# Gericom/MobiclipDecoder

Measured on AMD Instinct MI355X. Metric: decoded Mpixels/s @ 640x480 P-frames, higher is better.
Workload: dtype u8

## Files before the change

### mobiclipdecoder_amd/csrc/mobi_kernels.hip

```cpp
#include <hip/hip_runtime.h>
#include <stdint.h>
#include <stdlib.h>

#include <type_traits>

#include "mobi_cmd.h"
#include "mobi_kernels.h"
#include "mobi_recon_math.h"
#include "mobi_tile.h"

namespace {

enum { TP = 32 };

__device__ __forceinline__ void wave_sync() { __builtin_amdgcn_fence(__ATOMIC_ACQ_REL, "wavefront"); }

struct Geo {
  int width, height, stride, mbw, lg;
  __device__ __forceinline__ int owner_luma(int a) const {
    if (a < 0) return -1;
    const int row = a >> lg, col = a & (stride - 1);
    if (col >= width || row >= height) return -1;
    return (row >> 4) * mbw + (col >> 4);
  }
// ... 235 lines not shown
  const uint32_t pA[2] = {*(const uint32_t *)waA, *(const uint32_t *)wbA}, pB[2] = {*(const uint32_t *)waB, *(const uint32_t *)wbB};
  uint32_t resA[2], resB[2];
#pragma unroll
  for (int h = 0; h < 2; h++) {
    uint32_t sat[4];
#pragma unroll
    for (int k = 0; k < 4; k++) {
      const s16x2 pp = __builtin_bit_cast(s16x2, __builtin_amdgcn_perm(pB[h], pA[h], 0x0c040c00u + (uint32_t)k * 0x00010001u));
      const s16x2 sum = __builtin_elementwise_add_sat(pp, out[4 * h + k] >> (short)6);
      lo = __builtin_elementwise_min(lo, sum);
      hi = __builtin_elementwise_max(hi, sum);
      sat[k] = sat_pk_u8(sum);
    }
    const uint32_t m01 = __builtin_amdgcn_perm(sat[1], sat[0], 0x05010400u), m23 = __builtin_amdgcn_perm(sat[3], sat[2], 0x05010400u);
    resA[h] = __builtin_amdgcn_perm(m23, m01, 0x05040100u);
    resB[h] = __builtin_amdgcn_perm(m23, m01, 0x07060302u);
  }
  *(uint32_t *)waA = resA[0];
  *(uint32_t *)wbA = resA[1];
  if (actB) {
    *(uint32_t *)waB = resB[0];
    *(uint32_t *)wbB = resB[1];
  }
}
}

namespace {
enum {
  P_L = 0,
  P_C = 5120,
  P_C1 = 7680,
  P_BYTES = 10240,
  P_OUT = 0,
  P_COEF = 3072,
  P_TILE = 72,
#ifndef MOBI_PK_PAIRS
#define MOBI_PK_PAIRS 12
#endif
  P_PAIRS = MOBI_PK_PAIRS,
  P_ROUND = 22,
  P_SUM = P_COEF + P_PAIRS * P_TILE * 4,
  P_SC = 9728,
  P_TAB = 10048,
  P_INV = 9408
};
static_assert(P_COEF + P_ROUND * P_TILE * 4 <= P_INV && P_INV + 192 <= P_SC && P_TAB + 192 <= P_BYTES && P_SUM + 192 <= P_INV, "inter LDS map");
__device__ __forceinline__ int out_px(int g, int R, int c) { return P_OUT + (R & 7) * 384 + (R >> 3) * 128 + ((g ^ (R & 7)) << 4) + c; }
__device__ __forceinline__ int out_y(int g, int R, int c) { return out_px(g, R, c); }
__device__ __forceinline__ int out_c(int g, int R, int pl, int x) { return out_px(g, 16 + R, pl * 8 + x); }
template <int N>
__device__ __forceinline__ void mc_rows(const uint32_t (&x0)[N + 1], const uint32_t (&x1)[N + 1], uint32_t sh, int phase, uint32_t *out) {
  const bool hor = (phase & 1) != 0, ver = (phase & 2) != 0;
  const uint32_t selA = 0x03020100u + sh * 0x01010101u, selB = hor ? selA + 0x01010101u : selA;
  const uint32_t Mh = hor ? 0xFEFEFEFEu : 0xFFFFFFFFu, Mv = ver ? 0xFEFEFEFEu : 0xFFFFFFFFu;
  uint32_t m[N + 1];
#pragma unroll
  for (int i = 0; i <= N; i++) {
    const uint32_t a = __builtin_amdgcn_perm(x1[i], x0[i], selA) & Mh, b = __builtin_amdgcn_perm(x1[i], x0[i], selB) & Mh;
    m[i] = __builtin_amdgcn_lerp(a, b, 0u) & Mv;
  }
#pragma unroll
  for (int i = 0; i < N; i++) out[i] = __builtin_amdgcn_lerp(m[i], ver ? m[i + 1] : m[i], 0u);
}
}

__device__ __forceinline__ unsigned long long prof_stamp() {
  __builtin_amdgcn_sched_barrier(0);
  asm volatile("" ::: "memory");
  const unsigned long long t = __builtin_readcyclecounter();
  asm volatile("" ::: "memory");
  __builtin_amdgcn_sched_barrier(0);
  return t;
}
template <int PROF, int CWR, int FUSED>
__device__ __forceinline__ void recon_inter_oct(const MobiReconArgs &A, uint8_t *L, uint32_t clip, uint32_t mby, uint32_t ox, int lane) {
  unsigned long long pt[7] = {0, 0, 0, 0, 0, 0, 0};
  if (PROF) pt[0] = prof_stamp();
  const uint32_t oi = clip * A.qpc + mby * A.qpr + ox;
  const uint32_t mbx0 = ox * 8, mbw = (uint32_t)A.mbw;
  const int nmb = (int)(mbw - mbx0 < 8 ? mbw - mbx0 : 8);
// ... 24 lines not shown
  const uint32_t inter_mask = (uint32_t)v64 & 0xFFu;
  const uint32_t multi_mask = (uint32_t)(v64 & __builtin_amdgcn_ballot_w64(nl > 1) & __builtin_amdgcn_ballot_w64(kind2 == 0)) & 0xFFu;
  if (inter_mask == 0) return;
  auto slot_off = [&](uint32_t ref) {
    int sl = A.ring_base - (int)ref;
    sl = sl < 0 ? sl + 6 : sl;
    return __umul24((uint32_t)sl, A.slot_bytes);
  };
  const uint32_t refA = slot_off((d.z >> 10) & 7), refB = slot_off((d.z >> 13) & 7);
  const int posA = (int)d.w, cposA = (int)d2.x, posB = (int)d2.y, cposB = (int)d2.z;
  const int phA = (d.z >> 16) & 3, cphA = (d.z >> 18) & 3, phB = (d.z >> 20) & 3, cphB = (d.z >> 22) & 3;
  const int topB = tb ? posB + (8 << lgS) : posB + 8, ctopB = tb ? cposB + (4 << lgS) : cposB + 4;
  const int wpx = lr ? 8 : 16, cwpx = lr ? 4 : 8;
  const int overA = max((posA & (S - 1)) + wpx + (phA & 1) - S, (cposA & (S - 1)) + cwpx + (cphA & 1) - (S >> 1));
  const int overB = max((topB & (S - 1)) + wpx + (phB & 1) - S, (ctopB & (S - 1)) + cwpx + (cphB & 1) - (S >> 1));
  const bool wrap = leaves && max(overA, kind2 != 0 ? overB : 0) > 0;
  const bool win = leaves && !wrap;
  const bool slow = multi || wrap;
  const uint32_t slow_mask = (uint32_t)__builtin_amdgcn_ballot_w64(slow) & 0xFFu;
  const bool any_lr = __builtin_amdgcn_ballot_w64(lr && win) != 0;
  {
    const int s = j & 3, ph = j >> 2;
    const bool colB = lr && s >= 2;
    const int sw = lr ? s & 1 : (s < 3 ? s : 2);
    auto chunk0 = [&](int top, uint32_t ref, uint32_t &u) {
      const int yo = (top >> lgS) & 1;
      const uint32_t lin = (uint32_t)(((top - (yo << lgS)) & ~7) + 8 * sw);
      u = lin >> (lgS + 1);
      return ref + mobi_ty_col(lin & (uint32_t)(S - 1));
    };
    uint32_t uP, uB;
    const uint32_t bP = chunk0(colB ? topB : posA, colB ? refB : refA, uP), bB = chunk0(topB, refB, uB);
    auto rowpart = [&](uint32_t v) { return ((v & ~7u) << (lgS + 1)) + (((v & 7u) + (v & 4u)) << 4); };
    const uint32_t vP = uP + (uint32_t)ph, vB = uB + (uint32_t)ph - 5u;
    const bool b2 = tb && ph, b34 = tb;
    const uint32_t base2 = b2 ? bB : bP, v2 = b2 ? vB : vP, base34 = b34 ? bB : bP, v34 = b34 ? vB : vP;
    const uint32_t v4 = (!tb && ph) ? v34 - 1u : v34;
    uint32_t o[5] = {bP + rowpart(vP), bP + rowpart(vP + 2), base2 + rowpart(v2 + 4), base34 + rowpart(v34 + 6), base34 + rowpart(v4 + 8)};
    if (win) {
#pragma unroll
      for (int t = 0; t < 5; t++) dma16_sv(clip_base, o[t], lds0 + P_L + t * 1024);
    }
    const int cs = j & 1, ch2 = j >> 1;
    auto cchunk0 = [&](int ctop, uint32_t ref, uint32_t &r) {
      const uint32_t lin = (uint32_t)((ctop & ~7) + 8 * cs);
      r = lin >> lgS;
      return ref + ysz + mobi_tc_x(lin & (uint32_t)(S - 1));
    };
    auto crowpart = [&](uint32_t r) { return ((r & ~7u) << lgS) + ((r & 7u) << 4); };
    uint32_t rA, rB;
    const uint32_t cA = cchunk0(cposA, refA, rA), cB = cchunk0(ctopB, refB, rB);
    const uint32_t qA = rA + (uint32_t)ch2, qB = rB + (uint32_t)ch2 - 5u;
    const bool cb1 = tb && ch2 >= 1;
    const uint32_t cbase1 = cb1 ? cB : cA, q1 = cb1 ? qB : qA, cbase2 = tb ? cB : cA;
    const uint32_t q2 = tb ? qB - (ch2 >= 2 ? (uint32_t)ch2 - 1u : 0u) : qA - (uint32_t)ch2;
    const uint32_t co[3] = {cA + crowpart(qA), cbase1 + crowpart(q1 + 4), cbase2 + crowpart(q2 + 8)};
    if (win) {
#pragma unroll
      for (int t = 0; t < 3; t++) dma16_sv(clip_base, co[t], lds0 + P_C + t * 1024);
    }
    if (any_lr) {
      const uint32_t q3 = rB + (uint32_t)ch2;
      if (lr && win) {
        dma16_sv(clip_base, cB + crowpart(q3), lds0 + P_C1);
        dma16_sv(clip_base, cB + crowpart(q3 + 4), lds0 + P_C1 + 1024);
        dma16_sv(clip_base, cB + crowpart(q3 + 8 - (uint32_t)ch2), lds0 + P_C1 + 2048);
      }
    }
  }
  MOBI_STOP(1);
  const int quant = __builtin_amdgcn_readfirstlane((int)((d.y >> 20) & 63));
  const uint32_t *pay = A.payload + (size_t)clip * A.pay_clip_words;
  const uint32_t *cw = pay + d.x + (multi ? MOBI_MV_CELLS : 0);
  uint32_t cwr[CWR];
#pragma unroll
  for (int k = 0; k < CWR; k++) asm volatile("" : "=v"(cwr[k]));
  const uint32_t *cwj = cw + j;
  const int left = (int)ncoef - j;
  if (left > 0) cwr[0] = cwj[0];
  if (__builtin_amdgcn_ballot_w64(ncoef > 8) != 0) {
#pragma unroll
    for (int k = 1; k < 4; k++)
      if (left > 8 * k) cwr[k] = cwj[8 * k];
    if (CWR > 4 && __builtin_amdgcn_ballot_w64(ncoef > 32) != 0) {
#pragma unroll
      for (int k = 4; k < CWR; k++)
        if (left > 8 * k) cwr[k] = cwj[8 * k];
    }
  }
  const int yrow = lane >> 2, yc4 = (lane & 3) * 4;
  const int cv = (lane >> 4) & 1, crow = (lane & 15) >> 1, cc4 = (lane & 1) * 4;
  uint32_t cell0 = 0, cell1 = 0;
  auto load_cell = [&](int gm, uint32_t &c) {
    if ((multi_mask >> gm) & 1) c = (pay + __builtin_amdgcn_readlane(d.x, gm))[lane];
  };
  if (slow_mask) {
    load_cell(__builtin_ctz(slow_mask), cell0);
    const uint32_t m2 = slow_mask & (slow_mask - 1);
    if (m2) load_cell(__builtin_ctz(m2), cell1);
// ... 120 lines not shown
    const bool cBl = (tb && ch) || (lr && qc);
    const int ctop = cBl ? ctopB : cposA, cph = cBl ? cphB : cphA;
    const int cxo = ctop & 7, d0 = (cxo + (lr ? 0 : 4 * qc)) >> 2, d1 = d0 + 1;
    const int base = ((lr && qc) ? P_C1 : P_C) + ((tb && ch) ? 5 : 4 * ch) * 256 + g * 16 + pl * 8;
    const int a0 = base + (d0 >> 1) * 128 + (d0 & 1) * 4, a1 = base + (d1 >> 1) * 128 + (d1 & 1) * 4;
    uint32_t x0[5], x1[5];
#pragma unroll
    for (int k = 0; k < 5; k++) { x0[k] = lds32(L, a0 + k * 256); x1[k] = lds32(L, a1 + k * 256); }
    mc_rows<4>(x0, x1, (uint32_t)cxo & 3u, cph, mcv + 8);
  }
  MOBI_STOP(4);
  asm volatile("s_waitcnt lgkmcnt(0)" ::: "memory");
  if (lane < MOBI_SCALE_STRIDE / 4) MOBI_DMA16((const uint8_t *)(A.scale + quant * MOBI_SCALE_STRIDE) + lane * 16, L + P_SC, 0);
  {
    const bool rB = tb && rr, qB = lr && q >= 2;
    const int ytop = rB || qB ? topB : posA, yph = rB || qB ? phB : phA;
    const int yo = (ytop >> lgS) & 1, xo = ytop & 7;
    const int d0 = (xo + 4 * (qB ? q - 2 : q)) >> 2, d1 = d0 + 1;
    const int base = P_L + (rB ? 5 : 4 * rr) * 512 + g * 16 + (qB ? 256 : 0);
    const int a0 = base + (d0 >> 1) * 128 + (d0 & 1) * 4, a1 = base + (d1 >> 1) * 128 + (d1 & 1) * 4;
    const int ev = yo * 8, od = yo ? 512 : 8;
    uint32_t x0[9], x1[9];
#pragma unroll
    for (int k = 0; k < 9; k++) {
      const int o = (k >> 1) * 512 + ((k & 1) ? od : ev);
      x0[k] = lds32(L, a0 + o);
      x1[k] = lds32(L, a1 + o);
    }
    mc_rows<8>(x0, x1, (uint32_t)xo & 3u, yph, mcv);
  }
  MOBI_STOP(5);
  wave_sync();
  {
    const int by = P_OUT + rr * 128 + (g << 4) + 4 * q, bc = P_OUT + 256 + ch * (4 * 384) + ((g << 4) ^ (ch << 6)) + pl * 8 + 4 * qc;
#pragma unroll
    for (int k = 0; k < 8; k++) *(uint32_t *)(L + ((by ^ (k << 4)) + k * 384)) = mcv[k];
#pragma unroll
    for (int k = 0; k < 4; k++) *(uint32_t *)(L + ((bc ^ (k << 4)) + k * 384)) = mcv[8 + k];
  }
  if (PROF) pt[3] = prof_stamp();
  MOBI_STOP(6);
  if (slow_mask) {
    asm volatile("s_waitcnt vmcnt(0)" ::: "memory");
    deep_finish(__builtin_ctz(slow_mask), D0);
    uint32_t mm = slow_mask & (slow_mask - 1);
    bool second = true;
    while (mm) {
      const int gm = __builtin_ctz(mm);
      mm &= mm - 1;
      uint32_t cell = cell1;
      if (!second) load_cell(gm, cell);
      second = false;
      Deep Dn;
      deep_fetch(Dn, gm, cell);
      asm volatile("" ::: "memory");
      deep_finish(gm, Dn);
    }
  }
  if (PROF) pt[4] = prof_stamp();
  MOBI_STOP(7);

  asm volatile("s_waitcnt vmcnt(0)" ::: "memory");
  wave_sync();
  if (m_lo | m_hi) {
    const uint32_t m8_lo = m_lo & t_lo, m8_hi = m_hi & t_hi, m4_lo = m_lo & ~t_lo, m4_hi = m_hi & ~t_hi;
    const int n8_lo = __builtin_popcount(m8_lo), n8 = n8_lo + __builtin_popcount(m8_hi);
    const int n4_lo = __builtin_popcount(m4_lo), first4 = (n8 + 1) & ~1, n_slots = first4 + n4_lo + __builtin_popcount(m4_hi);
    {
      const bool hi = lane >= 32;
      const int kk = lane & 31;
      if (((hi ? m_hi : m_lo) >> kk) & 1) {
        const bool is8 = ((hi ? t_hi : t_lo) >> kk) & 1;
        const uint32_t flip = is8 ? 0u : 0xFFFFFFFFu;
        const uint32_t mask = hi ? m_hi & (t_hi ^ flip) : m_lo & (t_lo ^ flip);
        const int first = (is8 ? 0 : first4) + (hi ? (is8 ? n8_lo : n4_lo) : 0);
        const int slot = first + __builtin_popcount(mask & ((1u << kk) - 1u));
        const int a = lane >> 3;
        const uint32_t K = (uint32_t)((a < 4 ? a >> 1 : 2) * 128 + (a & 1) * 8);
        *(uint32_t *)(L + P_TAB + 4 * slot) = ((uint32_t)(lane & 7) << 4) | ((uint32_t)lane << 8) | (K << 16);
        *(uint32_t *)(L + P_INV + 4 * lane) = (uint32_t)((slot >> 1) * (P_TILE * 4) + (slot & 1) * 2) | ((uint32_t)slot << 13) | ((is8 ? 0x0FCu : 0x13Cu) << 23);
      }
      if (lane < 48) *(uint32_t *)(L + P_SUM + 4 * lane) = 0u;
    }
    wave_sync();
    MOBI_STOP(8);
    s16x2 lo = {0, 0}, hi = {0, 0};
    const int r = lane & 7, grp = lane >> 3;
    auto scatter_all = [&](auto pk, int base) {
      constexpr bool PK = decltype(pk)::value;
      const int base_off = PK ? (base >> 1) * (P_TILE * 4) : 0;
      auto scatter = [&](uint32_t e) {
        const uint32_t t = e & 0x1FF, t4 = t << 2, p4 = t4 & 0xFCu, kk4 = ((t >> 6) * 8 + (uint32_t)g) << 2;
        const int level = (int32_t)e >> 16;
        const uint32_t inv = lds32(L, P_INV + (int)kk4);
        const int scale = (int)lds32(L, P_SC + (int)((t4 | 0x100u) & (inv >> 23)));
        const int v = __mul24(scale, level);
        if (PK) {
          const uint32_t off = (inv & 0x1FFFu) - (uint32_t)base_off;
          if (off < (uint32_t)(P_PAIRS * P_TILE * 4)) *(int16_t *)(L + P_COEF + off + p4) = (int16_t)v;
          if (base == 0) {
            const int av = v < 0 ? -v : v;
            __hip_atomic_fetch_add((uint32_t *)(L + P_SUM + kk4), (uint32_t)(av > 0xFFFF ? 0xFFFF : av), __ATOMIC_RELAXED, __HIP_MEMORY_SCOPE_WAVEFRONT);
          }
        } else {
          const int slot = (int)((inv >> 13) & 0x7Fu) - base;
          if ((unsigned)slot < (unsigned)P_ROUND) *(int *)(L + P_COEF + slot * (P_TILE * 4) + p4) = v;
        }
      };
#pragma unroll
      for (int k = 0; k < CWR; k++) {
        int lf = left;
        asm volatile("" : "+v"(lf));
        const bool mine = lf > 8 * k;
        if (k && __builtin_amdgcn_ballot_w64(mine) == 0) break;
        uint32_t e = cwr[k];
        asm volatile("" : "+v"(e));
        if (mine) scatter(e);
      }
      for (uint32_t i = 8u * CWR + (uint32_t)j; __builtin_amdgcn_ballot_w64(i < ncoef) != 0; i += 64) {
        uint32_t tw[8];
#pragma unroll
        for (int k = 0; k < 8; k++) tw[k] = i + 8u * k < ncoef ? cw[i + 8u * k] : 0u;
#pragma unroll
        for (int k = 0; k < 8; k++)
          if (i + 8u * k < ncoef) scatter(tw[k]);
      }
    };
    auto zero_tiles = [&](int n_tiles) {
      const uint4 z = uint4{0, 0, 0, 0};
      for (int o = lane * 16; o < n_tiles * P_TILE * 4; o += 1024) *(uint4 *)(L + P_COEF + o) = z;
    };
    const int s4 = r >> 1, rowa4 = (s4 >> 1) * 4 + (r & 1) * 2, cola4 = (s4 & 1) * 4;
    const int Ca8 = P_OUT + r * 384, Cb8 = Ca8 + 4, x8 = r << 4;
    const int Ca4 = P_OUT + rowa4 * 384 + cola4, Cb4 = P_OUT + (rowa4 + 1) * 384 + cola4, xa4 = rowa4 << 4, xb4 = (rowa4 + 1) << 4;
    bool wide = false;
    for (int base = 0; base < n_slots && !wide; base += 2 * P_PAIRS) {
      zero_tiles(n_slots - base < 2 * P_PAIRS ? (n_slots - base + 1) >> 1 : P_PAIRS);
      wave_sync();
      scatter_all(std::true_type{}, base);
      wave_sync();
      if (base == 0) {
        const uint32_t sm = lane < 48 ? lds32(L, P_SUM + 4 * lane) : 0u;
        if (__builtin_amdgcn_ballot_w64(sm > (uint32_t)MOBI_PK_LIMIT) != 0) { wide = true; break; }
      }
      MOBI_STOP(9);
      for (int sub = 0; sub < P_PAIRS && base + 2 * sub < n_slots; sub += 8) {
        const int slot0 = base + 2 * (sub + grp);
        const bool act = sub + grp < P_PAIRS && slot0 < n_slots, is8g = slot0 < first4;
        const bool actB = slot0 + 1 < n_slots && slot0 + 1 != n8;
        uint32_t *tile = (uint32_t *)(L + P_COEF) + P_TILE * (sub + grp);
        if (act) idct_pass1_pk(tile, is8g, r);
        wave_sync();
        MOBI_STOP(10);
        if (act) {
          const uint32_t recA = lds32(L, P_TAB + 4 * slot0), recB = actB ? lds32(L, P_TAB + 4 * slot0 + 4) : recA;
          const int Ca = is8g ? Ca8 : Ca4, Cb = is8g ? Cb8 : Cb4, xa = is8g ? x8 : xa4, xb = is8g ? x8 : xb4;
          const int gA = (int)(recA & 0x70u), KA = (int)(recA >> 16), gB = (int)(recB & 0x70u), KB = (int)(recB >> 16);
          uint8_t *wa = L + (Ca + (gA ^ xa) + KA), *wb = L + (Cb + (gA ^ xb) + KA), *wc = L + (Ca + (gB ^ xa) + KB), *wd = L + (Cb + (gB ^ xb) + KB);
          idct_pass2_pk(tile, is8g, r, wa, wb, wc, wd, actB, lo, hi);
        }
        wave_sync();
        MOBI_STOP(11);
      }
    }
    if (wide) {
      const int hole = (n8 & 1) ? n8 : -1;
      for (int base = 0; base < n_slots; base += P_ROUND) {
        zero_tiles(n_slots - base < P_ROUND ? n_slots - base : P_ROUND);
        wave_sync();
        scatter_all(std::false_type{}, base);
        wave_sync();
        int *coef = (int *)(L + P_COEF);
        uint32_t recx[3];
        bool actx[3], is8x[3];
#pragma unroll
        for (int h = 0; h < 3; h++) {
          const int idx = base + 8 * h + grp;
          actx[h] = idx < n_slots && idx != hole && 8 * h + grp < P_ROUND;
          recx[h] = actx[h] ? lds32(L, P_TAB + 4 * idx) : 0u;
          is8x[h] = idx < n8;
        }
#pragma unroll
        for (int h = 0; h < 3; h++) {
          int *tile = coef + P_TILE * (8 * h + grp);
          if (actx[h]) idct_pass1(tile, tile, is8x[h], r);
        }
        wave_sync();
#pragma unroll
        for (int h = 0; h < 3; h++) {
          if (actx[h]) {
            const bool is8 = is8x[h];
            const int Ca = is8 ? Ca8 : Ca4, Cb = is8 ? Cb8 : Cb4, xa = is8 ? x8 : xa4, xb = is8 ? x8 : xb4;
            const int gg = (int)(recx[h] & 0x70u), KK = (int)(recx[h] >> 16);
            idct_pass2_q(coef + P_TILE * (8 * h + grp), is8, r, L + (Ca + (gg ^ xa) + KK), L + (Cb + (gg ^ xb) + KK), lo, hi);
          }
        }
        wave_sync();
      }
    }
    if (lo.x < -64 || lo.y < -64 || hi.x > 319 || hi.y > 319) atomicOr(&A.fault[clip], 1);
  }
  if (PROF) { asm volatile("s_waitcnt lgkmcnt(0)" ::: "memory"); pt[5] = prof_stamp(); }

  MOBI_STOP(12);
  __builtin_amdgcn_s_setprio(3);
  {
    uint8_t *y0 = clip_base + (uint32_t)A.ring_base * A.slot_bytes;
    uint8_t *ty0 = y0 + mobi_tile_y(mbx0, mby, lgS), *tc0 = y0 + ysz + mobi_tile_c(mbx0, mby, lgS);
    const bool full = nmb == 8;
    if (FUSED) {
#pragma unroll
      for (int it = 0; it < 2; it++) {
        const int i = lane + 64 * it, gq = i >> 4, quad = (i >> 2) & 3, R0 = (quad >> 1) * 8 + 2 * (i & 3), c0 = (quad & 1) * 8;
        const uint2 v0 = *(const uint2 *)(L + out_y(gq, R0, c0)), v1 = *(const uint2 *)(L + out_y(gq, R0 + 1, c0));
        const u32x4 v = {v0.x, v0.y, v1.x, v1.y};
        const uint8_t *dst = ty0 + i * 16;
        if ((inter_mask >> gq) & 1) asm volatile("global_store_dwordx4 %0, %1, off sc1\n\ts_nop 1" : : "v"(dst), "v"(v) : "memory");
      }
      {
        const int gq = lane >> 3, R = lane & 7;
        const uint4 c4 = *(const uint4 *)(L + out_c(gq, R, 0, 0));
        const u32x4 vc = {c4.x, c4.y, c4.z, c4.w};
        const uint8_t *dst = tc0 + lane * 16;
        if ((inter_mask >> gq) & 1) asm volatile("global_store_dwordx4 %0, %1, off sc1\n\ts_nop 1" : : "v"(dst), "v"(vc) : "memory");
      }
      asm volatile("s_waitcnt vmcnt(0)" ::: "memory");
      if (lane < 8 && ((inter_mask >> lane) & 1))
// ... 673 lines not shown
```

### mobiclipdecoder_amd/csrc/mobi_streamgen.cpp

```cpp
#include "mobi_streamgen.h"
#include "mobi_tables.h"

#include <algorithm>
#include <cstdlib>
#include <cstring>
#include <map>
#include <utility>
#include <vector>

namespace {

struct Rng {
  uint64_t s[4];
  static uint64_t splitmix(uint64_t &x) {
    uint64_t z = (x += 0x9E3779B97F4A7C15ull);
    z = (z ^ (z >> 30)) * 0xBF58476D1CE4E5B9ull;
    z = (z ^ (z >> 27)) * 0x94D049BB133111EBull;
    return z ^ (z >> 31);
  }
  explicit Rng(uint64_t seed) { for (auto &v : s) v = splitmix(seed); }
  static uint64_t rotl(uint64_t x, int k) { return (x << k) | (x >> (64 - k)); }
  uint64_t next() {
    uint64_t r = rotl(s[1] * 5, 7) * 9, t = s[1] << 17;
    s[2] ^= s[0]; s[3] ^= s[1]; s[1] ^= s[2]; s[0] ^= s[3]; s[2] ^= t; s[3] = rotl(s[3], 45);
// ... 433 lines not shown
        int r = (int)rng.below(1000);
        if (r < P.pm_intra) {
          bool sub = rng.chance(P.intra_sub_prob) && pinv[0].nbits[7];
          int c = sub ? 7 : 6;
          bw.put(pinv[0].code[c], pinv[0].nbits[c]);
          if (sub) gen_intra_sub(mx, my); else gen_intra_full(mx, my);
          continue;
        }
        int t1 = P.pm_intra + P.pm_skip, t2 = t1 + P.pm_split1, t3 = t2 + P.pm_deep;
        if (r < t1 && mv_ok(x, y, 16, 16, predx, predy)) gen_leaf(0, x, y, 16, 16, io, true);
        else if (r >= t1 && r < t2) gen_pblock(0, 0, x, y, io, 1, true);
        else if (r >= t2 && r < t3) gen_pblock(0, 0, x, y, io, 3 + (int)rng.below(4), true);
        else gen_leaf(0, x, y, 16, 16, io, false);
        gen_p_residual();
      }
    }
  }

  typedef std::map<std::pair<int, int>, std::vector<mobi_gen_script_tok>> TokMap;
  void put_block_scripted(const std::vector<mobi_gen_script_tok> &t) {
    int prev = -1;
    for (size_t i = 0; i < t.size(); i++) {
      Sym s{i + 1 == t.size(), t[i].pos - prev - 1, t[i].level};
      put_sym(s, std::abs(t[i].level) >= 32 ? 3 : t[i].form);
      prev = t[i].pos;
    }
  }
  void put_area_scripted(const mobi_gen_script_mb &m, int k, const TokMap &tm) {
    if ((m.t8 >> k) & 1) { bw.put(1, 1); put_block_scripted(tm.at({m.mb, 4 * k})); return; }
    const int m4 = m.cbp4[k];
    if (m.intra) bw.ue(m4 == 0 ? 2 : inv_cbp4_intra[m4]); else bw.ue(inv_cbp4_inter[m4]);
    for (int q = 0; q < 4; q++) if ((m4 >> q) & 1) put_block_scripted(tm.at({m.mb, 4 * k + q}));
  }
  void gen_pframe_scripted(int dq, const std::map<int, mobi_gen_script_mb> &mbs, const TokMap &tm) {
    bw.put(0, 1);
    bw.se(dq);
    if (ver == 0) { if (quant == 0) setup_quant(0); else if (dq) setup_quant(quant + dq); }
    else if (dq) setup_quant(quant + dq);
    vlc_table = 0;
    for (int mb = 0; mb < mbw * mbh; mb++) {
      mobi_gen_script_mb none;
      memset(&none, 0, sizeof(none));
      none.mb = mb;
      auto it = mbs.find(mb);
      const mobi_gen_script_mb &m = it == mbs.end() ? none : it->second;
      if (m.intra) {
        bw.put(pinv[0].code[6], pinv[0].nbits[6]);
        bw.ue(inv_cbp_intra[m.cbp]);
        bw.put(3, 3);
        for (int k = 0; k < 4; k++) if ((m.cbp >> k) & 1) put_area_scripted(m, k, tm);
        bw.put(3, 3);
        for (int k = 4; k < 6; k++) if ((m.cbp >> k) & 1) put_area_scripted(m, k, tm);
      } else {
        bw.put(pinv[0].code[1], pinv[0].nbits[1]);
        bw.se(0);
        bw.se(0);
        bw.ue(inv_cbp_inter[m.cbp]);
        for (int k = 0; k < 6; k++) if ((m.cbp >> k) & 1) put_area_scripted(m, k, tm);
      }
    }
  }
};

}

extern "C" void mobi_gen_default_params(mobi_gen_params *p, int config, uint64_t seed) {
  memset(p, 0, sizeof(*p));
  p->seed = seed;
  p->n_frames = 33;
  p->quantizer = 25;
  p->pm_skip = 150; p->pm_split1 = 200; p->pm_deep = 50; p->pm_intra = 50; p->pm_multiref = 50;
  p->mv_range = 16;
  p->cbp_prob = 300; p->t8_prob = 800; p->dense_prob = 0; p->max_coefs = 6; p->scan_span = 16;
  p->intra_sub_prob = 500; p->plane_prob = 300; p->intra_dc_only = 0;
  p->edge_mode = 0; p->escape_prob = 20; p->qdelta_prob = 0; p->table1_prob = 0;
  switch (config) {
    case 'A': p->width = 256; p->height = 192; p->version = 1; break;
    case 'C': p->width = 848; p->height = 480; p->version = 2; p->mv_range = 64; p->dense_prob = 300; p->quantizer = 16; break;
    case 'B': default: p->width = 640; p->height = 480; p->version = 2; break;
  }
}

extern "C" int64_t mobi_gen_clip(const mobi_gen_params *p, uint8_t *out, size_t cap, uint32_t *frame_off) {
  if (!p || p->width == 0 || p->height == 0 || (p->width & 15) || (p->height & 15) || p->width > 1024) return -1;
  if (p->version != 1 && p->version != 2) return -1;
  if (p->quantizer < 12 || p->quantizer > 52 || p->n_frames < 1) return -1;
  Gen g(*p);
  size_t total = 0;
  for (int f = 0; f < p->n_frames; f++) {
    if (frame_off) frame_off[f] = (uint32_t)total;
    g.bw = BitWriter();
    bool iframe = (f == 0) || (p->iframe_interval > 0 && f % p->iframe_interval == 0);
    if (iframe) g.gen_iframe(); else g.gen_pframe();
    g.bw.align();
    g.frames_done++;
    size_t n = g.bw.out.size();
    if (out && total + n <= cap) memcpy(out + total, g.bw.out.data(), n);
    total += n;
  }
  if (frame_off) frame_off[p->n_frames] = (uint32_t)total;
  if (total > cap) return -(int64_t)total;
  return (int64_t)total;
}

extern "C" int64_t mobi_gen_clip_scripted(const mobi_gen_params *p, const int32_t *frame_qdelta, const mobi_gen_script_mb *mbs, int32_t n_mbs,
                                          const mobi_gen_script_tok *toks, int32_t n_toks, uint8_t *out, size_t cap, uint32_t *frame_off) {
  if (!p || p->width == 0 || p->height == 0 || (p->width & 15) || (p->height & 15) || p->width > 1024) return -1;
  if (p->version != 1 && p->version != 2) return -1;
  if (p->quantizer < 12 || p->quantizer > 52 || p->n_frames < 1) return -1;
  if (n_mbs < 0 || n_toks < 0 || (n_mbs && !mbs) || (n_toks && !toks)) return -1;
  const int n_mb = (int)(p->width / 16) * (int)(p->height / 16);
  auto is_iframe = [&](int f) { return f == 0 || (p->iframe_interval > 0 && f % p->iframe_interval == 0); };
  std::vector<std::map<int, mobi_gen_script_mb>> fm(p->n_frames);
  std::vector<Gen::TokMap> ft(p->n_frames);
  for (int i = 0; i < n_mbs; i++) {
    const mobi_gen_script_mb &m = mbs[i];
    if (m.frame < 0 || m.frame >= p->n_frames || is_iframe(m.frame) || m.mb < 0 || m.mb >= n_mb || (m.intra & ~1) || (m.cbp & ~63) || (m.t8 & ~63)) return -1;
    for (int k = 0; k < 6; k++)
      if (((m.cbp >> k) & 1) && !((m.t8 >> k) & 1) && (m.cbp4[k] < (m.intra ? 0 : 1) || m.cbp4[k] > 15)) return -1;
    if (!fm[m.frame].emplace(m.mb, m).second) return -1;
  }
  for (int i = 0; i < n_toks; i++) {
    const mobi_gen_script_tok &t = toks[i];
    if (t.frame < 0 || t.frame >= p->n_frames || t.block < 0 || t.block >= 24 || t.level == 0 || t.level < -2048 || t.level > 2047 || t.form < 0 || t.form > 3) return -1;
    auto it = fm[t.frame].find(t.mb);
    if (it == fm[t.frame].end()) return -1;
    const mobi_gen_script_mb &m = it->second;
    const int k = t.block >> 2, q = t.block & 3;
    if (!((m.cbp >> k) & 1)) return -1;
    const bool is8 = (m.t8 >> k) & 1;
    if (is8 ? q != 0 : !((m.cbp4[k] >> q) & 1)) return -1;
    if (t.pos < 0 || t.pos >= (is8 ? 64 : 16)) return -1;
    ft[t.frame][{t.mb, t.block}].push_back(t);
  }
  for (int f = 0; f < p->n_frames; f++) {
    for (auto &kv : ft[f]) {
      auto &v = kv.second;
      std::sort(v.begin(), v.end(), [](const mobi_gen_script_tok &a, const mobi_gen_script_tok &b) { return a.pos < b.pos; });
      for (size_t i = 1; i < v.size(); i++) if (v[i].pos == v[i - 1].pos) return -1;
    }
    for (auto &kv : fm[f]) {
      const mobi_gen_script_mb &m = kv.second;
      for (int k = 0; k < 6; k++) {
        if (!((m.cbp >> k) & 1)) continue;
        const int m4 = ((m.t8 >> k) & 1) ? 1 : m.cbp4[k];
        for (int q = 0; q < 4; q++) if (((m4 >> q) & 1) && !ft[f].count({m.mb, 4 * k + q})) return -1;
      }
    }
  }
  Gen g(*p);
  size_t total = 0;
  long q = p->quantizer;
  for (int f = 0; f < p->n_frames; f++) {
    if (frame_off) frame_off[f] = (uint32_t)total;
    g.bw = BitWriter();
    if (is_iframe(f)) g.gen_iframe();
    else {
      const int dq = frame_qdelta ? frame_qdelta[f] : 0;
      q += dq;
      if (q < 12 || q > 52) return -1;
      g.gen_pframe_scripted(dq, fm[f], ft[f]);
    }
    g.bw.align();
    g.frames_done++;
    size_t n = g.bw.out.size();
    if (out && total + n <= cap) memcpy(out + total, g.bw.out.data(), n);
    total += n;
  }
  if (frame_off) frame_off[p->n_frames] = (uint32_t)total;
  if (total > cap) return -(int64_t)total;
  return (int64_t)total;
}
```

### mobiclipdecoder_amd/csrc/mobi_streamgen.h

```cpp
#ifndef MOBI_STREAMGEN_H
#define MOBI_STREAMGEN_H
#include <stddef.h>
#include <stdint.h>

#ifdef __cplusplus
extern "C" {
#endif

typedef struct mobi_gen_params {
  uint32_t width, height;
  int32_t version;
  uint64_t seed;
  int32_t n_frames;
  int32_t quantizer;
  int32_t iframe_interval;
  int32_t pm_skip;
  int32_t pm_split1;
  int32_t pm_deep;
  int32_t pm_intra;
  int32_t pm_multiref;
  int32_t mv_range;
  int32_t cbp_prob;
  int32_t t8_prob;
  int32_t dense_prob;
// ... 2 lines not shown
  int32_t intra_sub_prob;
  int32_t plane_prob;
  int32_t intra_dc_only;
  int32_t edge_mode;
  int32_t escape_prob;
  int32_t qdelta_prob;
  int32_t table1_prob;
  int32_t lowfreq_prob;
} mobi_gen_params;

void mobi_gen_default_params(mobi_gen_params *p, int config, uint64_t seed);

int64_t mobi_gen_clip(const mobi_gen_params *p, uint8_t *out, size_t cap, uint32_t *frame_off);

typedef struct mobi_gen_script_mb {
  int32_t frame;
  int32_t mb;
  int32_t intra;
  int32_t cbp;
  int32_t t8;
  int32_t cbp4[6];
} mobi_gen_script_mb;
typedef struct mobi_gen_script_tok {
  int32_t frame, mb;
  int32_t block;
  int32_t pos;
  int32_t level;
  int32_t form;
} mobi_gen_script_tok;

int64_t mobi_gen_clip_scripted(const mobi_gen_params *p, const int32_t *frame_qdelta, const mobi_gen_script_mb *mbs, int32_t n_mbs,
                               const mobi_gen_script_tok *toks, int32_t n_toks, uint8_t *out, size_t cap, uint32_t *frame_off);

#ifdef __cplusplus
}
#endif
#endif
```

### mobiclipdecoder_amd/streamgen.py

```python
import ctypes as C
import os

import numpy as np

_HERE = os.path.dirname(os.path.abspath(__file__))
_LIB = None


class GenParams(C.Structure):
    _fields_ = [
        ("width", C.c_uint32), ("height", C.c_uint32), ("version", C.c_int32), ("seed", C.c_uint64),
        ("n_frames", C.c_int32), ("quantizer", C.c_int32), ("iframe_interval", C.c_int32),
        ("pm_skip", C.c_int32), ("pm_split1", C.c_int32), ("pm_deep", C.c_int32), ("pm_intra", C.c_int32),
        ("pm_multiref", C.c_int32), ("mv_range", C.c_int32), ("cbp_prob", C.c_int32), ("t8_prob", C.c_int32),
        ("dense_prob", C.c_int32), ("max_coefs", C.c_int32), ("scan_span", C.c_int32),
        ("intra_sub_prob", C.c_int32), ("plane_prob", C.c_int32), ("intra_dc_only", C.c_int32),
        ("edge_mode", C.c_int32), ("escape_prob", C.c_int32), ("qdelta_prob", C.c_int32), ("table1_prob", C.c_int32),
        ("lowfreq_prob", C.c_int32),
    ]


def _lib():
    global _LIB
    if _LIB is None:
        path = os.path.join(_HERE, "libmobi_streamgen.so")
        if not os.path.exists(path):
            raise ImportError(f"{path} missing: run `python -m mobiclipdecoder_amd.build` (or __graft_entry__.build())")
        lib = C.CDLL(path)
        lib.mobi_gen_default_params.argtypes = [C.POINTER(GenParams), C.c_int, C.c_uint64]
        lib.mobi_gen_default_params.restype = None
        lib.mobi_gen_clip.argtypes = [C.POINTER(GenParams), C.c_void_p, C.c_size_t, C.c_void_p]
        lib.mobi_gen_clip.restype = C.c_int64
        lib.mobi_gen_clip_scripted.argtypes = [C.POINTER(GenParams), C.c_void_p, C.c_void_p, C.c_int32, C.c_void_p, C.c_int32, C.c_void_p, C.c_size_t, C.c_void_p]
        lib.mobi_gen_clip_scripted.restype = C.c_int64
        _LIB = lib
    return _LIB


BASE_SEED = 0x4D4F4249


def default_params(config="B", seed=BASE_SEED, **overrides):
    p = GenParams()
    _lib().mobi_gen_default_params(C.byref(p), ord(config), seed)
    for k, v in overrides.items():
        if not hasattr(p, k):
            raise AttributeError(k)
        setattr(p, k, v)
    return p


def generate_clip(p):
    lib = _lib()
    fo = np.zeros(p.n_frames + 1, np.uint32)
    need = lib.mobi_gen_clip(C.byref(p), None, 0, fo.ctypes.data)
    if need == -1:
        raise ValueError("bad generator parameters")
    n = -need if need < 0 else need
    buf = np.zeros(max(int(n), 2), np.uint8)
    got = lib.mobi_gen_clip(C.byref(p), buf.ctypes.data, buf.size, fo.ctypes.data)
    if got != n:
        raise RuntimeError(f"generator size mismatch {got} != {n}")
    return buf[: int(n)], fo


def generate_scripted(p, mbs, toks, qdelta=None):
    lib = _lib()
    mbs = np.ascontiguousarray(np.asarray(mbs, np.int32).reshape(-1, 11))
    toks = np.ascontiguousarray(np.asarray(toks, np.int32).reshape(-1, 6))
    qd = None if qdelta is None else np.ascontiguousarray(qdelta, np.int32)
    if qd is not None and qd.shape != (p.n_frames,):
        raise ValueError("qdelta needs one entry per frame")
    fo = np.zeros(p.n_frames + 1, np.uint32)
    args = (C.byref(p), None if qd is None else qd.ctypes.data, mbs.ctypes.data, len(mbs), toks.ctypes.data, len(toks))
    need = lib.mobi_gen_clip_scripted(*args, None, 0, fo.ctypes.data)
    if need == -1:
        raise ValueError("bad generator parameters or script")
    n = -need if need < 0 else need
    buf = np.zeros(max(int(n), 2), np.uint8)
    got = lib.mobi_gen_clip_scripted(*args, buf.ctypes.data, buf.size, fo.ctypes.data)
    if got != n:
        raise RuntimeError(f"generator size mismatch {got} != {n}")
    return buf[: int(n)], fo
```

Baseline: 1.011 million.

## Use padded output pitch in inter LDS tile and simplify reference row addressing

Replaces the XOR-swizzled 384-byte output row layout in LDS with a linear layout at a padded 400-byte pitch, which removes the XOR math on the MC store and IDCT pass-2 write paths. The slot table now packs the precomputed column offset, so pass 2 can compute its write addresses with a single add. The luma and chroma reference-row DMA address generation is rewritten around step helpers built on umul24, cutting per-lane ALU. The stream generator also gains scripted motion vectors for testing. The padding enlarges the LDS map, and bank conflicts may change relative to the swizzle.

```diff
diff --git a/mobiclipdecoder_amd/csrc/mobi_kernels.hip b/mobiclipdecoder_amd/csrc/mobi_kernels.hip
--- a/mobiclipdecoder_amd/csrc/mobi_kernels.hip
+++ b/mobiclipdecoder_amd/csrc/mobi_kernels.hip
@@ -291,7 +291,8 @@
   P_C1 = 7680,
   P_BYTES = 10240,
   P_OUT = 0,
-  P_COEF = 3072,
+  P_PITCH = 400,
+  P_COEF = 3200,
   P_TILE = 72,
 #ifndef MOBI_PK_PAIRS
 #define MOBI_PK_PAIRS 12
@@ -301,10 +302,11 @@
   P_SUM = P_COEF + P_PAIRS * P_TILE * 4,
   P_SC = 9728,
   P_TAB = 10048,
-  P_INV = 9408
+  P_INV = 9536
 };
-static_assert(P_COEF + P_ROUND * P_TILE * 4 <= P_INV && P_INV + 192 <= P_SC && P_TAB + 192 <= P_BYTES && P_SUM + 192 <= P_INV, "inter LDS map");
-__device__ __forceinline__ int out_px(int g, int R, int c) { return P_OUT + (R & 7) * 384 + (R >> 3) * 128 + ((g ^ (R & 7)) << 4) + c; }
+static_assert(P_OUT + 7 * P_PITCH + 384 <= P_COEF && P_COEF + P_ROUND * P_TILE * 4 <= P_INV && P_INV + 192 <= P_SC && P_SC + 320 <= P_TAB && P_TAB + 192 <= P_BYTES && P_SUM + 192 <= P_INV, "inter LDS map");
+static_assert(23 * P_TILE * 4 + 2 < (1 << 13) && (P_PITCH & 15) == 0, "P_INV's offset field (48 slots); 16-byte reads of the output rows");
+__device__ __forceinline__ int out_px(int g, int R, int c) { return P_OUT + (R & 7) * P_PITCH + (R >> 3) * 128 + (g << 4) + c; }
 __device__ __forceinline__ int out_y(int g, int R, int c) { return out_px(g, R, c); }
 __device__ __forceinline__ int out_c(int g, int R, int pl, int x) { return out_px(g, 16 + R, pl * 8 + x); }
 template <int N>
@@ -395,11 +397,22 @@
     uint32_t uP, uB;
     const uint32_t bP = chunk0(colB ? topB : posA, colB ? refB : refA, uP), bB = chunk0(topB, refB, uB);
     auto rowpart = [&](uint32_t v) { return ((v & ~7u) << (lgS + 1)) + (((v & 7u) + (v & 4u)) << 4); };
-    const uint32_t vP = uP + (uint32_t)ph, vB = uB + (uint32_t)ph - 5u;
-    const bool b2 = tb && ph, b34 = tb;
-    const uint32_t base2 = b2 ? bB : bP, v2 = b2 ? vB : vP, base34 = b34 ? bB : bP, v34 = b34 ? vB : vP;
-    const uint32_t v4 = (!tb && ph) ? v34 - 1u : v34;
-    uint32_t o[5] = {bP + rowpart(vP), bP + rowpart(vP + 2), base2 + rowpart(v2 + 4), base34 + rowpart(v34 + 6), base34 + rowpart(v4 + 8)};
+    const uint32_t Tm = (16u << lgS) - 256u;
+    auto rows3 = [&](uint32_t base, uint32_t v, uint32_t (&r)[3]) {
+      uint32_t h = (v >> 2) & 1u, e = (v >> 1) & 1u;
+      asm volatile("" : "+v"(h), "+v"(e));
+      const uint32_t dm = __umul24(h, Tm) + 64u;
+      r[0] = base + rowpart(v);
+      r[1] = __umul24(e, dm) + r[0] + 32u;
+      r[2] = r[0] + 64u + dm;
+    };
+    const uint32_t vP = uP + (uint32_t)ph;
+    uint32_t r1[3], r2[3];
+    rows3(bP, vP, r1);
+    rows3(tb ? bB : bP, tb ? uB + 1u - (uint32_t)ph : vP + 4u, r2);
+    const bool early = tb && !ph;
+    const bool short2 = tb != (ph != 0);
+    const uint32_t o[5] = {r1[0], r1[1], early ? r1[2] : r2[0], early ? r2[0] : r2[1], short2 ? r2[1] : r2[2]};
     if (win) {
 #pragma unroll
       for (int t = 0; t < 5; t++) dma16_sv(clip_base, o[t], lds0 + P_L + t * 1024);
@@ -413,11 +426,18 @@
     auto crowpart = [&](uint32_t r) { return ((r & ~7u) << lgS) + ((r & 7u) << 4); };
     uint32_t rA, rB;
     const uint32_t cA = cchunk0(cposA, refA, rA), cB = cchunk0(ctopB, refB, rB);
-    const uint32_t qA = rA + (uint32_t)ch2, qB = rB + (uint32_t)ch2 - 5u;
-    const bool cb1 = tb && ch2 >= 1;
-    const uint32_t cbase1 = cb1 ? cB : cA, q1 = cb1 ? qB : qA, cbase2 = tb ? cB : cA;
-    const uint32_t q2 = tb ? qB - (ch2 >= 2 ? (uint32_t)ch2 - 1u : 0u) : qA - (uint32_t)ch2;
-    const uint32_t co[3] = {cA + crowpart(qA), cbase1 + crowpart(q1 + 4), cbase2 + crowpart(q2 + 8)};
+    const uint32_t Tc = 8u << lgS, Tcm = Tc - 128u;
+    auto cstep4 = [&](uint32_t r) {
+      uint32_t h = (r >> 2) & 1u;
+      asm volatile("" : "+v"(h));
+      return __umul24(h, Tcm) + 64u;
+    };
+    const uint32_t qA = rA + (uint32_t)ch2;
+    const uint32_t c0 = cA + crowpart(qA), cE = c0 + cstep4(qA);
+    const uint32_t cY = cB + crowpart(rB + (uint32_t)((ch2 + 3) & 3));
+    const uint32_t stB = cstep4(rB);
+    const uint32_t cYd = cY + (ch2 == 1 ? stB : 0u);
+    const uint32_t co[3] = {c0, (tb && ch2) ? cY : cE, tb ? cYd : (ch2 ? cE : c0 + Tc)};
     if (win) {
 #pragma unroll
       for (int t = 0; t < 3; t++) dma16_sv(clip_base, co[t], lds0 + P_C + t * 1024);
@@ -425,9 +445,10 @@
     if (any_lr) {
       const uint32_t q3 = rB + (uint32_t)ch2;
       if (lr && win) {
-        dma16_sv(clip_base, cB + crowpart(q3), lds0 + P_C1);
-        dma16_sv(clip_base, cB + crowpart(q3 + 4), lds0 + P_C1 + 1024);
-        dma16_sv(clip_base, cB + crowpart(q3 + 8 - (uint32_t)ch2), lds0 + P_C1 + 2048);
+        const uint32_t z0 = cB + crowpart(q3), z1 = z0 + cstep4(q3);
+        dma16_sv(clip_base, z0, lds0 + P_C1);
+        dma16_sv(clip_base, z1, lds0 + P_C1 + 1024);
+        dma16_sv(clip_base, ch2 ? z1 : z0 + Tc, lds0 + P_C1 + 2048);
       }
     }
   }
@@ -614,11 +635,11 @@
   MOBI_STOP(5);
   wave_sync();
   {
-    const int by = P_OUT + rr * 128 + (g << 4) + 4 * q, bc = P_OUT + 256 + ch * (4 * 384) + ((g << 4) ^ (ch << 6)) + pl * 8 + 4 * qc;
-#pragma unroll
-    for (int k = 0; k < 8; k++) *(uint32_t *)(L + ((by ^ (k << 4)) + k * 384)) = mcv[k];
-#pragma unroll
-    for (int k = 0; k < 4; k++) *(uint32_t *)(L + ((bc ^ (k << 4)) + k * 384)) = mcv[8 + k];
+    const int by = out_y(g, 8 * rr, 4 * q), bc = out_c(g, 4 * ch, pl, 4 * qc);
+#pragma unroll
+    for (int k = 0; k < 8; k++) *(uint32_t *)(L + (by + k * P_PITCH)) = mcv[k];
+#pragma unroll
+    for (int k = 0; k < 4; k++) *(uint32_t *)(L + (bc + k * P_PITCH)) = mcv[8 + k];
   }
   if (PROF) pt[3] = prof_stamp();
   MOBI_STOP(6);
@@ -659,7 +680,7 @@
         const int slot = first + __builtin_popcount(mask & ((1u << kk) - 1u));
         const int a = lane >> 3;
         const uint32_t K = (uint32_t)((a < 4 ? a >> 1 : 2) * 128 + (a & 1) * 8);
-        *(uint32_t *)(L + P_TAB + 4 * slot) = ((uint32_t)(lane & 7) << 4) | ((uint32_t)lane << 8) | (K << 16);
+        *(uint32_t *)(L + P_TAB + 4 * slot) = ((uint32_t)lane << 8) | ((K + ((uint32_t)(lane & 7) << 4)) << 16);
         *(uint32_t *)(L + P_INV + 4 * lane) = (uint32_t)((slot >> 1) * (P_TILE * 4) + (slot & 1) * 2) | ((uint32_t)slot << 13) | ((is8 ? 0x0FCu : 0x13Cu) << 23);
       }
       if (lane < 48) *(uint32_t *)(L + P_SUM + 4 * lane) = 0u;
@@ -713,8 +734,7 @@
       for (int o = lane * 16; o < n_tiles * P_TILE * 4; o += 1024) *(uint4 *)(L + P_COEF + o) = z;
     };
     const int s4 = r >> 1, rowa4 = (s4 >> 1) * 4 + (r & 1) * 2, cola4 = (s4 & 1) * 4;
-    const int Ca8 = P_OUT + r * 384, Cb8 = Ca8 + 4, x8 = r << 4;
-    const int Ca4 = P_OUT + rowa4 * 384 + cola4, Cb4 = P_OUT + (rowa4 + 1) * 384 + cola4, xa4 = rowa4 << 4, xb4 = (rowa4 + 1) << 4;
+    const int Ca8 = P_OUT + r * P_PITCH, Ca4 = P_OUT + rowa4 * P_PITCH + cola4;
     bool wide = false;
     for (int base = 0; base < n_slots && !wide; base += 2 * P_PAIRS) {
       zero_tiles(n_slots - base < 2 * P_PAIRS ? (n_slots - base + 1) >> 1 : P_PAIRS);
@@ -736,9 +756,8 @@
         MOBI_STOP(10);
         if (act) {
           const uint32_t recA = lds32(L, P_TAB + 4 * slot0), recB = actB ? lds32(L, P_TAB + 4 * slot0 + 4) : recA;
-          const int Ca = is8g ? Ca8 : Ca4, Cb = is8g ? Cb8 : Cb4, xa = is8g ? x8 : xa4, xb = is8g ? x8 : xb4;
-          const int gA = (int)(recA & 0x70u), KA = (int)(recA >> 16), gB = (int)(recB & 0x70u), KB = (int)(recB >> 16);
-          uint8_t *wa = L + (Ca + (gA ^ xa) + KA), *wb = L + (Cb + (gA ^ xb) + KA), *wc = L + (Ca + (gB ^ xa) + KB), *wd = L + (Cb + (gB ^ xb) + KB);
+          const int Ca = is8g ? Ca8 : Ca4, dab = is8g ? 4 : P_PITCH;
+          uint8_t *wa = L + (Ca + (int)(recA >> 16)), *wb = wa + dab, *wc = L + (Ca + (int)(recB >> 16)), *wd = wc + dab;
           idct_pass2_pk(tile, is8g, r, wa, wb, wc, wd, actB, lo, hi);
         }
         wave_sync();
@@ -772,9 +791,8 @@
         for (int h = 0; h < 3; h++) {
           if (actx[h]) {
             const bool is8 = is8x[h];
-            const int Ca = is8 ? Ca8 : Ca4, Cb = is8 ? Cb8 : Cb4, xa = is8 ? x8 : xa4, xb = is8 ? x8 : xb4;
-            const int gg = (int)(recx[h] & 0x70u), KK = (int)(recx[h] >> 16);
-            idct_pass2_q(coef + P_TILE * (8 * h + grp), is8, r, L + (Ca + (gg ^ xa) + KK), L + (Cb + (gg ^ xb) + KK), lo, hi);
+            uint8_t *wa = L + ((is8 ? Ca8 : Ca4) + (int)(recx[h] >> 16));
+            idct_pass2_q(coef + P_TILE * (8 * h + grp), is8, r, wa, wa + (is8 ? 4 : P_PITCH), lo, hi);
           }
         }
         wave_sync();
diff --git a/mobiclipdecoder_amd/csrc/mobi_streamgen.cpp b/mobiclipdecoder_amd/csrc/mobi_streamgen.cpp
--- a/mobiclipdecoder_amd/csrc/mobi_streamgen.cpp
+++ b/mobiclipdecoder_amd/csrc/mobi_streamgen.cpp
@@ -489,19 +489,61 @@
     if (m.intra) bw.ue(m4 == 0 ? 2 : inv_cbp4_intra[m4]); else bw.ue(inv_cbp4_inter[m4]);
     for (int q = 0; q < 4; q++) if ((m4 >> q) & 1) put_block_scripted(tm.at({m.mb, 4 * k + q}));
   }
-  void gen_pframe_scripted(int dq, const std::map<int, mobi_gen_script_mb> &mbs, const TokMap &tm) {
+  bool put_leaf_scripted(int s, int x, int y, int w, int h, int io, int ref, int dx, int dy) {
+    const int nref = frames_done < 5 ? frames_done : 5;
+    if (ref < 1 || ref > nref || !pinv[s].nbits[ref] || std::abs(dx) > 63 || std::abs(dy) > 63 || !mv_ok(x, y, w, h, dx, dy)) return false;
+    bw.put(pinv[s].code[ref], pinv[s].nbits[ref]);
+    bw.se(dx - predx);
+    bw.se(dy - predy);
+    mvc[io] = dx; mvc[io + 1] = dy;
+    return true;
+  }
+  bool put_motion_scripted(const mobi_gen_script_mv &v, int x, int y, int io) {
+    switch (v.shape) {
+      case 0: return put_leaf_scripted(0, x, y, 16, 16, io, v.ref[0], v.dx[0], v.dy[0]);
+      case 1:
+        if (!pinv[0].nbits[8]) return false;
+        bw.put(pinv[0].code[8], pinv[0].nbits[8]);
+        return put_leaf_scripted(1, x, y, 16, 8, io, v.ref[0], v.dx[0], v.dy[0]) && put_leaf_scripted(1, x, y + 8, 16, 8, io, v.ref[1], v.dx[1], v.dy[1]);
+      case 2:
+        if (!pinv[0].nbits[9]) return false;
+        bw.put(pinv[0].code[9], pinv[0].nbits[9]);
+        return put_leaf_scripted(4, x, y, 8, 16, io, v.ref[0], v.dx[0], v.dy[0]) && put_leaf_scripted(4, x + 8, y, 8, 16, io, v.ref[1], v.dx[1], v.dy[1]);
+      case 3:
+        if (!pinv[0].nbits[8] || !pinv[1].nbits[9]) return false;
+        bw.put(pinv[0].code[8], pinv[0].nbits[8]);
+        for (int half = 0; half < 2; half++) {
+          bw.put(pinv[1].code[9], pinv[1].nbits[9]);
+          for (int k = 0; k < 2; k++)
+            if (!put_leaf_scripted(5, x + 8 * k, y + 8 * half, 8, 8, io, v.ref[2 * half + k], v.dx[2 * half + k], v.dy[2 * half + k])) return false;
+        }
+        return true;
+    }
+    return false;
+  }
+  bool gen_pframe_scripted(int dq, const std::map<int, mobi_gen_script_mb> &mbs, const TokMap &tm, const std::map<int, mobi_gen_script_mv> &mvs) {
     bw.put(0, 1);
     bw.se(dq);
     if (ver == 0) { if (quant == 0) setup_quant(0); else if (dq) setup_quant(quant + dq); }
     else if (dq) setup_quant(quant + dq);
     vlc_table = 0;
+    std::fill(mvc.begin(), mvc.end(), 0);
     for (int mb = 0; mb < mbw * mbh; mb++) {
       mobi_gen_script_mb none;
       memset(&none, 0, sizeof(none));
       none.mb = mb;
       auto it = mbs.find(mb);
       const mobi_gen_script_mb &m = it == mbs.end() ? none : it->second;
+      const int mx = mb % mbw, my = mb / mbw;
+      int io = 2 * mx;
+      int a[3] = {mvc[io], mvc[io + 2], mvc[io + 4]}, b[3] = {mvc[io + 1], mvc[io + 3], mvc[io + 5]};
+      auto med = [](int *v) { if (v[0] > v[1]) std::swap(v[0], v[1]); if (v[1] > v[2]) std::swap(v[1], v[2]); if (v[0] > v[1]) std::swap(v[0], v[1]); return v[1]; };
+      predx = med(a); predy = med(b);
+      io += 2;
+      mvc[io] = 0; mvc[io + 1] = 0;
+      auto mv = mvs.find(mb);
       if (m.intra) {
+        if (mv != mvs.end()) return false;
         bw.put(pinv[0].code[6], pinv[0].nbits[6]);
         bw.ue(inv_cbp_intra[m.cbp]);
         bw.put(3, 3);
@@ -509,13 +551,18 @@
         bw.put(3, 3);
         for (int k = 4; k < 6; k++) if ((m.cbp >> k) & 1) put_area_scripted(m, k, tm);
       } else {
-        bw.put(pinv[0].code[1], pinv[0].nbits[1]);
-        bw.se(0);
-        bw.se(0);
+        if (mv != mvs.end()) {
+          if (!put_motion_scripted(mv->second, mx * 16, my * 16, io)) return false;
+        } else {
+          bw.put(pinv[0].code[1], pinv[0].nbits[1]);
+          bw.se(0 - predx);
+          bw.se(0 - predy);
+        }
         bw.ue(inv_cbp_inter[m.cbp]);
         for (int k = 0; k < 6; k++) if ((m.cbp >> k) & 1) put_area_scripted(m, k, tm);
       }
     }
+    return true;
   }
 };
 
@@ -562,10 +609,16 @@
 
 extern "C" int64_t mobi_gen_clip_scripted(const mobi_gen_params *p, const int32_t *frame_qdelta, const mobi_gen_script_mb *mbs, int32_t n_mbs,
                                           const mobi_gen_script_tok *toks, int32_t n_toks, uint8_t *out, size_t cap, uint32_t *frame_off) {
+  return mobi_gen_clip_scripted_mv(p, frame_qdelta, mbs, n_mbs, toks, n_toks, nullptr, 0, out, cap, frame_off);
+}
+
+extern "C" int64_t mobi_gen_clip_scripted_mv(const mobi_gen_params *p, const int32_t *frame_qdelta, const mobi_gen_script_mb *mbs, int32_t n_mbs,
+                                             const mobi_gen_script_tok *toks, int32_t n_toks, const mobi_gen_script_mv *mvs, int32_t n_mvs,
+                                             uint8_t *out, size_t cap, uint32_t *frame_off) {
   if (!p || p->width == 0 || p->height == 0 || (p->width & 15) || (p->height & 15) || p->width > 1024) return -1;
   if (p->version != 1 && p->version != 2) return -1;
   if (p->quantizer < 12 || p->quantizer > 52 || p->n_frames < 1) return -1;
-  if (n_mbs < 0 || n_toks < 0 || (n_mbs && !mbs) || (n_toks && !toks)) return -1;
+  if (n_mbs < 0 || n_toks < 0 || n_mvs < 0 || (n_mbs && !mbs) || (n_toks && !toks) || (n_mvs && !mvs)) return -1;
   const int n_mb = (int)(p->width / 16) * (int)(p->height / 16);
   auto is_iframe = [&](int f) { return f == 0 || (p->iframe_interval > 0 && f % p->iframe_interval == 0); };
   std::vector<std::map<int, mobi_gen_script_mb>> fm(p->n_frames);
@@ -576,6 +629,12 @@
     for (int k = 0; k < 6; k++)
       if (((m.cbp >> k) & 1) && !((m.t8 >> k) & 1) && (m.cbp4[k] < (m.intra ? 0 : 1) || m.cbp4[k] > 15)) return -1;
     if (!fm[m.frame].emplace(m.mb, m).second) return -1;
+  }
+  std::vector<std::map<int, mobi_gen_script_mv>> fv(p->n_frames);
+  for (int i = 0; i < n_mvs; i++) {
+    const mobi_gen_script_mv &v = mvs[i];
+    if (v.frame < 0 || v.frame >= p->n_frames || is_iframe(v.frame) || v.mb < 0 || v.mb >= n_mb || v.shape < 0 || v.shape > 3) return -1;
+    if (!fv[v.frame].emplace(v.mb, v).second) return -1;
   }
   for (int i = 0; i < n_toks; i++) {
     const mobi_gen_script_tok &t = toks[i];
@@ -616,7 +675,7 @@
       const int dq = frame_qdelta ? frame_qdelta[f] : 0;
       q += dq;
       if (q < 12 || q > 52) return -1;
-      g.gen_pframe_scripted(dq, fm[f], ft[f]);
+      if (!g.gen_pframe_scripted(dq, fm[f], ft[f], fv[f])) return -1;
     }
     g.bw.align();
     g.frames_done++;
diff --git a/mobiclipdecoder_amd/csrc/mobi_streamgen.h b/mobiclipdecoder_amd/csrc/mobi_streamgen.h
--- a/mobiclipdecoder_amd/csrc/mobi_streamgen.h
+++ b/mobiclipdecoder_amd/csrc/mobi_streamgen.h
@@ -58,6 +58,15 @@
 int64_t mobi_gen_clip_scripted(const mobi_gen_params *p, const int32_t *frame_qdelta, const mobi_gen_script_mb *mbs, int32_t n_mbs,
                                const mobi_gen_script_tok *toks, int32_t n_toks, uint8_t *out, size_t cap, uint32_t *frame_off);
 
+typedef struct mobi_gen_script_mv {
+  int32_t frame, mb;
+  int32_t shape;
+  int32_t ref[4], dx[4], dy[4];
+} mobi_gen_script_mv;
+int64_t mobi_gen_clip_scripted_mv(const mobi_gen_params *p, const int32_t *frame_qdelta, const mobi_gen_script_mb *mbs, int32_t n_mbs,
+                                  const mobi_gen_script_tok *toks, int32_t n_toks, const mobi_gen_script_mv *mvs, int32_t n_mvs,
+                                  uint8_t *out, size_t cap, uint32_t *frame_off);
+
 #ifdef __cplusplus
 }
 #endif
diff --git a/mobiclipdecoder_amd/streamgen.py b/mobiclipdecoder_amd/streamgen.py
--- a/mobiclipdecoder_amd/streamgen.py
+++ b/mobiclipdecoder_amd/streamgen.py
@@ -33,6 +33,8 @@
         lib.mobi_gen_clip.restype = C.c_int64
         lib.mobi_gen_clip_scripted.argtypes = [C.POINTER(GenParams), C.c_void_p, C.c_void_p, C.c_int32, C.c_void_p, C.c_int32, C.c_void_p, C.c_size_t, C.c_void_p]
         lib.mobi_gen_clip_scripted.restype = C.c_int64
+        lib.mobi_gen_clip_scripted_mv.argtypes = [C.POINTER(GenParams), C.c_void_p, C.c_void_p, C.c_int32, C.c_void_p, C.c_int32, C.c_void_p, C.c_int32, C.c_void_p, C.c_size_t, C.c_void_p]
+        lib.mobi_gen_clip_scripted_mv.restype = C.c_int64
         _LIB = lib
     return _LIB
 
@@ -64,7 +66,7 @@
     return buf[: int(n)], fo
 
 
-def generate_scripted(p, mbs, toks, qdelta=None):
+def generate_scripted(p, mbs, toks, qdelta=None, motion=None):
     lib = _lib()
     mbs = np.ascontiguousarray(np.asarray(mbs, np.int32).reshape(-1, 11))
     toks = np.ascontiguousarray(np.asarray(toks, np.int32).reshape(-1, 6))
@@ -72,13 +74,14 @@
     if qd is not None and qd.shape != (p.n_frames,):
         raise ValueError("qdelta needs one entry per frame")
     fo = np.zeros(p.n_frames + 1, np.uint32)
-    args = (C.byref(p), None if qd is None else qd.ctypes.data, mbs.ctypes.data, len(mbs), toks.ctypes.data, len(toks))
-    need = lib.mobi_gen_clip_scripted(*args, None, 0, fo.ctypes.data)
+    mv = np.ascontiguousarray(np.asarray([] if motion is None else motion, np.int32).reshape(-1, 15))
+    args = (C.byref(p), None if qd is None else qd.ctypes.data, mbs.ctypes.data, len(mbs), toks.ctypes.data, len(toks), mv.ctypes.data, len(mv))
+    need = lib.mobi_gen_clip_scripted_mv(*args, None, 0, fo.ctypes.data)
     if need == -1:
         raise ValueError("bad generator parameters or script")
     n = -need if need < 0 else need
     buf = np.zeros(max(int(n), 2), np.uint8)
-    got = lib.mobi_gen_clip_scripted(*args, buf.ctypes.data, buf.size, fo.ctypes.data)
+    got = lib.mobi_gen_clip_scripted_mv(*args, buf.ctypes.data, buf.size, fo.ctypes.data)
     if got != n:
         raise RuntimeError(f"generator size mismatch {got} != {n}")
     return buf[: int(n)], fo
```

After: 1.025 million (median of 6 runs). 1.4% higher.
